# Foxhead-Studio/InsTaG

Hardware: AMD Instinct MI355X
Metric: train-step frames/sec @512x512, 100k Gaussians (higher is better)
Workload: dtype f32; 1 GPU; C3: train_face step, 100k Gaussians + 6 grid encodes + UMF/PMF motion nets (DeepSpeech feats), 512x512, SH degree 1, image + attention map in one raster pass, L1+DSSIM, Adam; targets = uniform noise (SURVEY 8d); gaussians=100000, sh_degree=1, parallelism=dp1, ranks_reported_by_backend=1, execution=hipGraph replay, timing=one window of 1714 steps after 5 warm-up steps

## Files before the change

### instag_amd/csrc/ssim.hip

```cpp
#include "common.hpp"
#include "device_math.hpp"

namespace instag {
namespace {

constexpr int TS = 16;
constexpr int RAD = 5;
constexpr int HS = TS + 2 * RAD;
constexpr float C1 = 0.01f * 0.01f;
constexpr float C2 = 0.03f * 0.03f;

__device__ constexpr float GW[11] = {0.0010283801f, 0.0075987581f, 0.0360007721f, 0.1093606895f, 0.2130055377f,
                                     0.2660117249f, 0.2130055377f, 0.1093606895f, 0.0360007721f, 0.0075987581f,
                                     0.0010283801f};

__global__ void __launch_bounds__(256)
l1_ssim_forward_kernel(const float* __restrict__ img1, const float* __restrict__ img2, int H, int W,
                       float* __restrict__ maps, float* __restrict__ part_ssim, float* __restrict__ part_l1) {
  __shared__ float s_x[HS][HS + 1], s_y[HS][HS + 1];
  __shared__ float s_h[5][HS][TS + 1];
  __shared__ float s_red[4];
  const int c = blockIdx.z;
  const int x0 = blockIdx.x * TS, y0 = blockIdx.y * TS;
  const size_t plane = (size_t)H * W;
  const float* p1 = img1 + c * plane;
  const float* p2 = img2 + c * plane;
  for (int i = threadIdx.x; i < HS * HS; i += 256) {
    const int ly = i / HS, lx = i - ly * HS;
    const int gy = y0 + ly - RAD, gx = x0 + lx - RAD;
    const bool in = gy >= 0 && gy < H && gx >= 0 && gx < W;
    s_x[ly][lx] = in ? p1[(size_t)gy * W + gx] : 0.f;
    s_y[ly][lx] = in ? p2[(size_t)gy * W + gx] : 0.f;
  }
  __syncthreads();
  for (int i = threadIdx.x; i < HS * TS; i += 256) {
    const int ly = i / TS, lx = i - ly * TS;
    float a = 0.f, b = 0.f, aa = 0.f, bb = 0.f, ab = 0.f;
#pragma unroll
    for (int k = 0; k < 11; ++k) {
      const float xv = s_x[ly][lx + k], yv = s_y[ly][lx + k], w = GW[k];
      a += w * xv; b += w * yv; aa += w * xv * xv; bb += w * yv * yv; ab += w * xv * yv;
    }
    s_h[0][ly][lx] = a; s_h[1][ly][lx] = b; s_h[2][ly][lx] = aa; s_h[3][ly][lx] = bb; s_h[4][ly][lx] = ab;
  }
  __syncthreads();
  const int tx = threadIdx.x & 15, ty = threadIdx.x >> 4;
  const int gx = x0 + tx, gy = y0 + ty;
  const bool inside = gx < W && gy < H;
  float mu1 = 0.f, mu2 = 0.f, e11 = 0.f, e22 = 0.f, e12 = 0.f;
#pragma unroll
  for (int k = 0; k < 11; ++k) {
    const float w = GW[k];
    mu1 += w * s_h[0][ty + k][tx]; mu2 += w * s_h[1][ty + k][tx];
    e11 += w * s_h[2][ty + k][tx]; e22 += w * s_h[3][ty + k][tx]; e12 += w * s_h[4][ty + k][tx];
  }
  float ssim_v = 0.f, l1_v = 0.f;
  if (inside) {
    const float mu1s = mu1 * mu1, mu2s = mu2 * mu2, mu12 = mu1 * mu2;
    const float s11 = e11 - mu1s, s22 = e22 - mu2s, s12 = e12 - mu12;
    const float A1 = 2.f * mu12 + C1, A2 = 2.f * s12 + C2, B1 = mu1s + mu2s + C1, B2 = s11 + s22 + C2;
    const float inv = 1.f / (B1 * B2);
    ssim_v = A1 * A2 * inv;
    const float dS_ds11 = -ssim_v / B2;
    const float dS_ds12 = 2.f * A1 * inv;
    const float dS_dmu1 = 2.f * mu2 * A2 * inv - 2.f * mu1 * ssim_v / B1 + dS_ds11 * (-2.f * mu1) + dS_ds12 * (-mu2);
    const size_t pix = (size_t)gy * W + gx;
    const size_t C3 = (size_t)gridDim.z * plane;
    maps[c * plane + pix] = dS_dmu1;
    maps[C3 + c * plane + pix] = dS_ds11;
    maps[2 * C3 + c * plane + pix] = dS_ds12;
    l1_v = fabsf(s_x[ty + RAD][tx + RAD] - s_y[ty + RAD][tx + RAD]);
  }
  const float bs = block_sum_256(ssim_v, s_red);
  __syncthreads();
  const float bl = block_sum_256(l1_v, s_red);
  if (threadIdx.x == 0) {
    const int bid = (blockIdx.z * gridDim.y + blockIdx.y) * gridDim.x + blockIdx.x;
    part_ssim[bid] = bs;
    part_l1[bid] = bl;
  }
}

__global__ void __launch_bounds__(256)
l1_ssim_backward_kernel(const float* __restrict__ img1, const float* __restrict__ img2,
                        const float* __restrict__ maps, const float* __restrict__ g_ssim,
                        const float* __restrict__ g_l1, int C, int H, int W, float* __restrict__ dimg1) {
  __shared__ float s_m[3][HS][HS + 1];
  __shared__ float s_h[3][HS][TS + 1];
  const int c = blockIdx.z;
  const int x0 = blockIdx.x * TS, y0 = blockIdx.y * TS;
  const size_t plane = (size_t)H * W;
  const size_t C3 = (size_t)C * plane;
  for (int i = threadIdx.x; i < HS * HS; i += 256) {
    const int ly = i / HS, lx = i - ly * HS;
    const int gy = y0 + ly - RAD, gx = x0 + lx - RAD;
    const bool in = gy >= 0 && gy < H && gx >= 0 && gx < W;
    const size_t o = c * plane + (size_t)gy * W + gx;
    s_m[0][ly][lx] = in ? maps[o] : 0.f;
    s_m[1][ly][lx] = in ? maps[C3 + o] : 0.f;
    s_m[2][ly][lx] = in ? maps[2 * C3 + o] : 0.f;
  }
  __syncthreads();
  for (int i = threadIdx.x; i < HS * TS; i += 256) {
    const int ly = i / TS, lx = i - ly * TS;
    float a = 0.f, b = 0.f, d = 0.f;
#pragma unroll
    for (int k = 0; k < 11; ++k) {
      const float w = GW[k];
      a += w * s_m[0][ly][lx + k]; b += w * s_m[1][ly][lx + k]; d += w * s_m[2][ly][lx + k];
    }
    s_h[0][ly][lx] = a; s_h[1][ly][lx] = b; s_h[2][ly][lx] = d;
  }
  __syncthreads();
  const int tx = threadIdx.x & 15, ty = threadIdx.x >> 4;
  const int gx = x0 + tx, gy = y0 + ty;
  if (gx >= W || gy >= H) return;
  float fm = 0.f, f11 = 0.f, f12 = 0.f;
#pragma unroll
  for (int k = 0; k < 11; ++k) {
    const float w = GW[k];
    fm += w * s_h[0][ty + k][tx]; f11 += w * s_h[1][ty + k][tx]; f12 += w * s_h[2][ty + k][tx];
  }
  const size_t pix = c * plane + (size_t)gy * W + gx;
  const float x = img1[pix], y = img2[pix];
  const float inv_n = 1.f / (float)C3;
  const float gs = g_ssim ? g_ssim[0] : 0.f, gl = g_l1 ? g_l1[0] : 0.f;
  const float diff = x - y;
  const float sgn = diff > 0.f ? 1.f : (diff < 0.f ? -1.f : 0.f);
  dimg1[pix] = inv_n * (gs * (fm + 2.f * x * f11 + y * f12) + gl * sgn);
}


struct FaceCfg {
  int H, W, flags;
  float w_dssim, w_alpha, w_hair, w_lips, w_extra;
};
constexpr int F_HAIR_BG = 1, F_ALPHA = 2, F_HAIR_ATTN = 4, F_LIPS = 8;
constexpr int F_MOUTH = 16;
constexpr int F_PLAIN = 32;

struct FaceIn {
  const float* image; const float* gt; const uint8_t* face; const uint8_t* hair; const uint8_t* mouth;
  const float* bg; const float* alpha; const float* attn; const int32_t* lips; const float* extra;
};

__device__ __forceinline__ bool in_lips(const FaceIn& in, int gy, int gx) {
  return gy >= in.lips[0] && gy < in.lips[1] && gx >= in.lips[2] && gx < in.lips[3];
}

__device__ __forceinline__ void face_pixel(const FaceCfg& cfg, const FaceIn& in, int c, size_t plane, size_t pix,
                                           float& x, float& y) {
  if (cfg.flags & F_PLAIN) {
    x = in.image[c * plane + pix];
    y = in.gt[c * plane + pix];
    return;
  }
  const float bgc = in.bg[c];
  if (cfg.flags & F_MOUTH) {
    const int gy = (int)(pix / (size_t)cfg.W), gx = (int)(pix - (size_t)gy * cfg.W);
    const bool mouth = in.mouth[pix] != 0, lips = in_lips(in, gy, gx);
    x = (lips != mouth) ? bgc : in.image[c * plane + pix];
    y = mouth ? in.gt[c * plane + pix] : bgc;
    return;
  }
  const bool hair = in.hair[pix] != 0, head = hair || in.face[pix] != 0, mouth = in.mouth[pix] != 0;
  const bool hair_bg = (cfg.flags & F_HAIR_BG) && hair;
  x = hair_bg ? bgc : in.image[c * plane + pix];
  y = (head && !mouth && !hair_bg) ? in.gt[c * plane + pix] : bgc;
}

__global__ void __launch_bounds__(256)
face_loss_forward_kernel(FaceCfg cfg, FaceIn in, float* __restrict__ maps, float* __restrict__ part) {
  __shared__ float s_x[HS][HS + 1], s_y[HS][HS + 1];
  __shared__ float s_h[5][HS][TS + 1];
  __shared__ float s_red[4];
  const int H = cfg.H, W = cfg.W;
  const int c = blockIdx.z;
  const int x0 = blockIdx.x * TS, y0 = blockIdx.y * TS;
  const size_t plane = (size_t)H * W;
  for (int i = threadIdx.x; i < HS * HS; i += 256) {
    const int ly = i / HS, lx = i - ly * HS;
    const int gy = y0 + ly - RAD, gx = x0 + lx - RAD;
    float xv = 0.f, yv = 0.f;
    if (gy >= 0 && gy < H && gx >= 0 && gx < W) face_pixel(cfg, in, c, plane, (size_t)gy * W + gx, xv, yv);
    s_x[ly][lx] = xv;
    s_y[ly][lx] = yv;
  }
  __syncthreads();
  for (int i = threadIdx.x; i < HS * TS; i += 256) {
    const int ly = i / TS, lx = i - ly * TS;
    float a = 0.f, b = 0.f, aa = 0.f, bb = 0.f, ab = 0.f;
#pragma unroll
    for (int k = 0; k < 11; ++k) {
      const float xv = s_x[ly][lx + k], yv = s_y[ly][lx + k], w = GW[k];
      a += w * xv; b += w * yv; aa += w * xv * xv; bb += w * yv * yv; ab += w * xv * yv;
    }
    s_h[0][ly][lx] = a; s_h[1][ly][lx] = b; s_h[2][ly][lx] = aa; s_h[3][ly][lx] = bb; s_h[4][ly][lx] = ab;
  }
  __syncthreads();
  const int tx = threadIdx.x & 15, ty = threadIdx.x >> 4;
  const int gx = x0 + tx, gy = y0 + ty;
  const bool inside = gx < W && gy < H;
  float mu1 = 0.f, mu2 = 0.f, e11 = 0.f, e22 = 0.f, e12 = 0.f;
#pragma unroll
  for (int k = 0; k < 11; ++k) {
    const float w = GW[k];
    mu1 += w * s_h[0][ty + k][tx]; mu2 += w * s_h[1][ty + k][tx];
    e11 += w * s_h[2][ty + k][tx]; e22 += w * s_h[3][ty + k][tx]; e12 += w * s_h[4][ty + k][tx];
  }
  float v[8] = {0.f, 0.f, 0.f, 0.f, 0.f, 0.f, 0.f, 0.f};
  if (inside) {
    const float mu1s = mu1 * mu1, mu2s = mu2 * mu2, mu12 = mu1 * mu2;
    const float s11 = e11 - mu1s, s22 = e22 - mu2s, s12 = e12 - mu12;
    const float A1 = 2.f * mu12 + C1, A2 = 2.f * s12 + C2, B1 = mu1s + mu2s + C1, B2 = s11 + s22 + C2;
    const float inv = 1.f / (B1 * B2);
    const float ssim_v = A1 * A2 * inv;
    const float dS_ds11 = -ssim_v / B2;
    const float dS_ds12 = 2.f * A1 * inv;
    const float dS_dmu1 = 2.f * mu2 * A2 * inv - 2.f * mu1 * ssim_v / B1 + dS_ds11 * (-2.f * mu1) + dS_ds12 * (-mu2);
    const size_t pix = (size_t)gy * W + gx;
    const size_t C3 = 3 * plane;
    maps[c * plane + pix] = dS_dmu1;
    maps[C3 + c * plane + pix] = dS_ds11;
    maps[2 * C3 + c * plane + pix] = dS_ds12;
    v[0] = ssim_v;
    v[1] = fabsf(s_x[ty + RAD][tx + RAD] - s_y[ty + RAD][tx + RAD]);
    if (c == 0) {
      const bool mouth_mode = (cfg.flags & F_MOUTH) != 0, plain = (cfg.flags & F_PLAIN) != 0;
      const bool hair = !mouth_mode && !plain && in.hair[pix] != 0;
      const bool head = plain ? false : (mouth_mode ? in_lips(in, gy, gx) : (hair || in.face[pix] != 0));
      if (cfg.flags & F_ALPHA) {
        const float a = in.alpha[pix];
        v[2] = head ? 1.f - a : 0.f;
        v[3] = head ? 0.f : a;
      }
      if ((cfg.flags & F_HAIR_ATTN) && hair) {
        v[4] = in.attn[plane + pix];
        v[5] = in.attn[pix];
        v[6] = 1.f;
      }
      if (cfg.flags & F_LIPS) {
        if (gy >= in.lips[0] && gy < in.lips[1] && gx >= in.lips[2] && gx < in.lips[3]) v[7] = in.attn[plane + pix];
      }
    }
  }
  const int tiles = gridDim.x * gridDim.y;
  const int tile = blockIdx.y * gridDim.x + blockIdx.x;
  const int nk = c == 0 ? 8 : 2;
#pragma unroll
  for (int k = 0; k < 8; ++k) {
    if (k >= nk) break;
    const float bsum = block_sum_256(v[k], s_red);
    __syncthreads();
    if (threadIdx.x == 0) {
      if (k < 2) part[(size_t)k * 3 * tiles + (size_t)c * tiles + tile] = bsum;
      else part[(size_t)6 * tiles + (size_t)(k - 2) * tiles + tile] = bsum;
    }
  }
}

__device__ __forceinline__ void face_loss_partial_sums(const float* __restrict__ part, int tiles,
                                                       const float* __restrict__ extra, int n_extra, float* s_sum,
                                                       int nwaves) {
  const int wave = threadIdx.x >> 6, lane = threadIdx.x & 63;
  for (int k = wave; k < 8; k += nwaves) {
    const float* p = k < 2 ? part + (size_t)k * 3 * tiles : part + (size_t)6 * tiles + (size_t)(k - 2) * tiles;
    const int n = k < 2 ? 3 * tiles : tiles;
    float acc = 0.f;
#pragma unroll 8
    for (int i = lane; i < n; i += 64) acc += p[i];
    acc = wave_sum(acc);
    if (lane == 0) s_sum[k] = acc;
    if (k == 7) {
      float e = 0.f;
      for (int i = lane; i < n_extra; i += 64) e += extra[i];
      e = wave_sum(e);
      if (lane == 0) s_sum[8] = e;
    }
  }
}

__device__ __forceinline__ float lips_inv_area(const FaceCfg& cfg, const int32_t* __restrict__ lips) {
  const int r0 = max(lips[0], 0), r1 = min(lips[1], cfg.H), c0 = max(lips[2], 0), c1 = min(lips[3], cfg.W);
  const float area = (float)max(r1 - r0, 0) * (float)max(c1 - c0, 0);
  return area > 0.f ? 1.f / area : 0.f;
}

__device__ __forceinline__ void face_loss_scalars(const FaceCfg& cfg, const float* s_sum, const int32_t* __restrict__ lips,
                                                  bool has_extra, float* __restrict__ out) {
  const float npix = (float)cfg.H * (float)cfg.W;
  const float l1 = s_sum[1] / (3.f * npix), ssim = s_sum[0] / (3.f * npix);
  float loss = l1 + cfg.w_dssim * (1.f - ssim);
  if (cfg.flags & F_ALPHA) loss += cfg.w_alpha * (s_sum[2] / npix + s_sum[3] / npix);
  const float inv_cnt = 1.f / fmaxf(s_sum[6], 1.f);
  if (cfg.flags & F_HAIR_ATTN) loss += cfg.w_hair * (s_sum[4] * inv_cnt + s_sum[5] * inv_cnt);
  float inv_area = 0.f;
  if (cfg.flags & F_LIPS) {
    inv_area = lips_inv_area(cfg, lips);
    loss += cfg.w_lips * s_sum[7] * inv_area;
  }
  if (has_extra) loss += cfg.w_extra * s_sum[8];
  out[0] = loss; out[1] = l1; out[2] = ssim; out[3] = inv_cnt; out[4] = inv_area;
}

__global__ void __launch_bounds__(512)
face_loss_finalize_kernel(FaceCfg cfg, const float* __restrict__ part, int tiles, const int32_t* __restrict__ lips,
                          const float* __restrict__ extra, int n_extra, float* __restrict__ out) {
  __shared__ float s_sum[9];
  face_loss_partial_sums(part, tiles, extra, n_extra, s_sum, 8);
  __syncthreads();
  if (threadIdx.x == 0) face_loss_scalars(cfg, s_sum, lips, extra != nullptr, out);
}

struct FaceFin {
  const float* part; int tiles; const float* extra; int n_extra; float* out;
};

__global__ void __launch_bounds__(256)
face_loss_backward_kernel(FaceCfg cfg, FaceIn in, const float* __restrict__ maps, const float* __restrict__ out,
                          const float* __restrict__ g_loss, const float* __restrict__ g_l1,
                          float* __restrict__ d_image, float* __restrict__ d_alpha, float* __restrict__ d_attn,
                          FaceFin fin) {
  __shared__ float s_m[3][HS][HS + 1];
  __shared__ float s_h[3][HS][TS + 1];
  __shared__ float s_sum[9];
  const int H = cfg.H, W = cfg.W;
  const int c = blockIdx.z;
  float inv_cnt = 0.f;
  if (fin.part != nullptr) {
    const bool first = blockIdx.x == 0 && blockIdx.y == 0 && c == 0;
    if (first) {
      face_loss_partial_sums(fin.part, fin.tiles, fin.extra, fin.n_extra, s_sum, 4);
      __syncthreads();
      if (threadIdx.x == 0) face_loss_scalars(cfg, s_sum, in.lips, fin.extra != nullptr, fin.out);
      inv_cnt = 1.f / fmaxf(s_sum[6], 1.f);
    } else if (c == 0 && (cfg.flags & F_HAIR_ATTN)) {
      const float* hp = fin.part + (size_t)6 * fin.tiles + (size_t)4 * fin.tiles;
      float acc = 0.f;
      for (int i = threadIdx.x; i < fin.tiles; i += 256) acc += hp[i];
      acc = block_sum_256(acc, s_sum);
      inv_cnt = 1.f / fmaxf(acc, 1.f);
    }
    __syncthreads();
  }
  const int x0 = blockIdx.x * TS, y0 = blockIdx.y * TS;
  const size_t plane = (size_t)H * W;
  const size_t C3 = 3 * plane;
  for (int i = threadIdx.x; i < HS * HS; i += 256) {
    const int ly = i / HS, lx = i - ly * HS;
    const int gy = y0 + ly - RAD, gx = x0 + lx - RAD;
    const bool inb = gy >= 0 && gy < H && gx >= 0 && gx < W;
    const size_t o = c * plane + (size_t)gy * W + gx;
    s_m[0][ly][lx] = inb ? maps[o] : 0.f;
    s_m[1][ly][lx] = inb ? maps[C3 + o] : 0.f;
    s_m[2][ly][lx] = inb ? maps[2 * C3 + o] : 0.f;
  }
  __syncthreads();
  for (int i = threadIdx.x; i < HS * TS; i += 256) {
    const int ly = i / TS, lx = i - ly * TS;
    float a = 0.f, b = 0.f, d = 0.f;
#pragma unroll
    for (int k = 0; k < 11; ++k) {
      const float w = GW[k];
      a += w * s_m[0][ly][lx + k]; b += w * s_m[1][ly][lx + k]; d += w * s_m[2][ly][lx + k];
    }
    s_h[0][ly][lx] = a; s_h[1][ly][lx] = b; s_h[2][ly][lx] = d;
  }
  __syncthreads();
  const int tx = threadIdx.x & 15, ty = threadIdx.x >> 4;
  const int gx = x0 + tx, gy = y0 + ty;
  if (gx >= W || gy >= H) return;
  float fm = 0.f, f11 = 0.f, f12 = 0.f;
#pragma unroll
  for (int k = 0; k < 11; ++k) {
    const float w = GW[k];
    fm += w * s_h[0][ty + k][tx]; f11 += w * s_h[1][ty + k][tx]; f12 += w * s_h[2][ty + k][tx];
  }
  const size_t pix = (size_t)gy * W + gx;
  float x, y;
  face_pixel(cfg, in, c, plane, pix, x, y);
  const float g = g_loss ? g_loss[0] : 0.f;
  const float gl = g + (g_l1 ? g_l1[0] : 0.f);
  const float gs = -cfg.w_dssim * g;
  const float diff = x - y;
  const float sgn = diff > 0.f ? 1.f : (diff < 0.f ? -1.f : 0.f);
  const bool mouth_mode = (cfg.flags & F_MOUTH) != 0, plain = (cfg.flags & F_PLAIN) != 0;
  const bool hair = !mouth_mode && !plain && in.hair[pix] != 0;
  const bool frozen = plain ? false
                            : (mouth_mode ? (in_lips(in, gy, gx) != (in.mouth[pix] != 0)) : ((cfg.flags & F_HAIR_BG) && hair));
  d_image[c * plane + pix] = frozen ? 0.f : (1.f / (float)C3) * (gs * (fm + 2.f * x * f11 + y * f12) + gl * sgn);
  if (c == 0) {
    const bool head = plain ? false : (mouth_mode ? in_lips(in, gy, gx) : (hair || in.face[pix] != 0));
    if (d_alpha) d_alpha[pix] = (cfg.flags & F_ALPHA) ? g * cfg.w_alpha / (float)plane * (head ? -1.f : 1.f) : 0.f;
    if (d_attn) {
      const float gh = ((cfg.flags & F_HAIR_ATTN) && hair) ? g * cfg.w_hair * (fin.part ? inv_cnt : out[3]) : 0.f;
      float gp = 0.f;
      if (cfg.flags & F_LIPS)
        if (gy >= in.lips[0] && gy < in.lips[1] && gx >= in.lips[2] && gx < in.lips[3])
          gp = g * cfg.w_lips * (fin.part ? lips_inv_area(cfg, in.lips) : out[4]);
      d_attn[pix] = gh;
      d_attn[plane + pix] = gh + gp;
      d_attn[2 * plane + pix] = 0.f;
    }
  }
}

}
}

using namespace instag;

extern "C" {

int instag_l1_ssim_num_partials(int32_t C, int32_t H, int32_t W) {
  return C * ((H + TS - 1) / TS) * ((W + TS - 1) / TS);
}

int instag_l1_ssim_forward(const float* img1, const float* img2, int32_t C, int32_t H, int32_t W, float* maps,
                           float* partial_ssim, float* partial_l1, instag_stream_t stream) {
  INSTAG_REQUIRE(img1 && img2 && maps && partial_ssim && partial_l1, "l1_ssim_forward: NULL tensor");
  INSTAG_REQUIRE(C >= 1 && C <= 65535 && H >= 1 && W >= 1, "l1_ssim_forward: bad shape");
  dim3 grid((W + TS - 1) / TS, (H + TS - 1) / TS, C);
  ProfScope p(K_LOSS_FWD, (hipStream_t)stream);
  l1_ssim_forward_kernel<<<grid, 256, 0, (hipStream_t)stream>>>(img1, img2, H, W, maps, partial_ssim, partial_l1);
  INSTAG_CHECK_LAUNCH();
  return INSTAG_OK;
}

int instag_l1_ssim_backward(const float* img1, const float* img2, const float* maps, const float* g_ssim,
                            const float* g_l1, int32_t C, int32_t H, int32_t W, float* dimg1,
                            instag_stream_t stream) {
  INSTAG_REQUIRE(img1 && img2 && maps && dimg1, "l1_ssim_backward: NULL tensor");
  INSTAG_REQUIRE(C >= 1 && C <= 65535 && H >= 1 && W >= 1, "l1_ssim_backward: bad shape");
  dim3 grid((W + TS - 1) / TS, (H + TS - 1) / TS, C);
  ProfScope p(K_LOSS_BWD, (hipStream_t)stream);
  l1_ssim_backward_kernel<<<grid, 256, 0, (hipStream_t)stream>>>(img1, img2, maps, g_ssim, g_l1, C, H, W, dimg1);
  INSTAG_CHECK_LAUNCH();
  return INSTAG_OK;
}

static int face_cfg(const instag_face_loss_cfg* c, FaceCfg* out) {
  INSTAG_REQUIRE(c, "face_loss: NULL config");
  INSTAG_REQUIRE(c->H >= 1 && c->W >= 1, "face_loss: bad image size");
  *out = FaceCfg{c->H, c->W, c->flags, c->w_dssim, c->w_alpha, c->w_attn_hair, c->w_attn_lips, c->w_extra};
  return INSTAG_OK;
}

int64_t instag_face_loss_num_partials(int32_t H, int32_t W) {
  return (int64_t)12 * ((H + TS - 1) / TS) * ((W + TS - 1) / TS);
}

static int face_loss_forward_impl(const instag_face_loss_cfg* cfg, const float* image, const float* gt,
                                  const uint8_t* face_mask, const uint8_t* hair_mask, const uint8_t* mouth_mask,
                                  const float* bg, const float* alpha, const float* attn, const int32_t* lips_rect,
                                  const float* extra, int32_t n_extra, float* maps, float* partials, float* out,
                                  bool finalize, instag_stream_t stream) {
  FaceCfg c;
  if (int rc = face_cfg(cfg, &c)) return rc;
  const bool mouth_mode = (c.flags & F_MOUTH) != 0;
  const bool plain = (c.flags & F_PLAIN) != 0;
  INSTAG_REQUIRE(image && gt && maps && partials && out, "face_loss_forward: NULL tensor");
  INSTAG_REQUIRE(plain || (mouth_mask && bg && (mouth_mode || (face_mask && hair_mask))), "face_loss_forward: NULL mask");
  INSTAG_REQUIRE(!plain || !(c.flags & ~F_PLAIN), "face_loss_forward: the plain mode takes no other term");
  INSTAG_REQUIRE(!mouth_mode || (lips_rect && !(c.flags & (F_HAIR_BG | F_HAIR_ATTN | F_LIPS))),
                 "face_loss_forward: the mouth mode needs lips_rect and none of the face-branch terms");
  INSTAG_REQUIRE(!(c.flags & F_ALPHA) || alpha, "face_loss_forward: alpha term without alpha");
  INSTAG_REQUIRE(!(c.flags & (F_HAIR_ATTN | F_LIPS)) || attn, "face_loss_forward: attention term without attn");
  INSTAG_REQUIRE(!(c.flags & F_LIPS) || lips_rect, "face_loss_forward: lips term without lips_rect");
  INSTAG_REQUIRE(extra == nullptr || n_extra >= 1, "face_loss_forward: n_extra must be >= 1");
  const FaceIn in{image, gt, face_mask, hair_mask, mouth_mask, bg, alpha, attn, lips_rect, extra};
  dim3 grid((c.W + TS - 1) / TS, (c.H + TS - 1) / TS, 3);
  {
    ProfScope p(K_LOSS_FWD, (hipStream_t)stream);
    face_loss_forward_kernel<<<grid, 256, 0, (hipStream_t)stream>>>(c, in, maps, partials);
    INSTAG_CHECK_LAUNCH();
  }
  if (!finalize) return INSTAG_OK;
  face_loss_finalize_kernel<<<1, 512, 0, (hipStream_t)stream>>>(c, partials, (int)(grid.x * grid.y), lips_rect, extra,
                                                              extra ? n_extra : 0, out);
  INSTAG_CHECK_LAUNCH();
  return INSTAG_OK;
}

int instag_face_loss_forward(const instag_face_loss_cfg* cfg, const float* image, const float* gt,
                             const uint8_t* face_mask, const uint8_t* hair_mask, const uint8_t* mouth_mask,
                             const float* bg, const float* alpha, const float* attn, const int32_t* lips_rect,
                             const float* extra, int32_t n_extra, float* maps, float* partials, float* out,
                             instag_stream_t stream) {
  return face_loss_forward_impl(cfg, image, gt, face_mask, hair_mask, mouth_mask, bg, alpha, attn, lips_rect, extra,
                                n_extra, maps, partials, out, true, stream);
}

int instag_face_loss_forward_deferred(const instag_face_loss_cfg* cfg, const float* image, const float* gt,
                                      const uint8_t* face_mask, const uint8_t* hair_mask, const uint8_t* mouth_mask,
                                      const float* bg, const float* alpha, const float* attn, const int32_t* lips_rect,
                                      const float* extra, int32_t n_extra, float* maps, float* partials,
                                      instag_stream_t stream) {
  INSTAG_REQUIRE(partials != nullptr, "face_loss_forward_deferred: NULL partials");
  float dummy = 0.f;
  return face_loss_forward_impl(cfg, image, gt, face_mask, hair_mask, mouth_mask, bg, alpha, attn, lips_rect, extra,
                                n_extra, maps, partials, &dummy, false, stream);
}

static int face_loss_backward_impl(const instag_face_loss_cfg* cfg, const float* image, const float* gt,
                                   const uint8_t* face_mask, const uint8_t* hair_mask, const uint8_t* mouth_mask,
                                   const float* bg, const int32_t* lips_rect, const float* maps, const float* out,
                                   const float* g_loss, const float* g_l1, float* d_image, float* d_alpha, float* d_attn,
                                   const FaceFin& fin, instag_stream_t stream) {
  FaceCfg c;
  if (int rc = face_cfg(cfg, &c)) return rc;
  const bool mouth_mode = (c.flags & F_MOUTH) != 0;
  const bool plain = (c.flags & F_PLAIN) != 0;
  INSTAG_REQUIRE(image && gt && maps && out && d_image, "face_loss_backward: NULL tensor");
  INSTAG_REQUIRE(plain || (mouth_mask && bg && (mouth_mode || (face_mask && hair_mask))), "face_loss_backward: NULL mask");
  INSTAG_REQUIRE(!mouth_mode || lips_rect, "face_loss_backward: the mouth mode needs lips_rect");
  INSTAG_REQUIRE(!(c.flags & F_LIPS) || lips_rect, "face_loss_backward: lips term without lips_rect");
  const FaceIn in{image, gt, face_mask, hair_mask, mouth_mask, bg, nullptr, nullptr, lips_rect, nullptr};
  dim3 grid((c.W + TS - 1) / TS, (c.H + TS - 1) / TS, 3);
  FaceFin f = fin;
  f.tiles = (int)(grid.x * grid.y);
  ProfScope p(K_LOSS_BWD, (hipStream_t)stream);
  face_loss_backward_kernel<<<grid, 256, 0, (hipStream_t)stream>>>(c, in, maps, out, g_loss, g_l1, d_image, d_alpha,
                                                                   d_attn, f);
  INSTAG_CHECK_LAUNCH();
  return INSTAG_OK;
}

int instag_face_loss_backward(const instag_face_loss_cfg* cfg, const float* image, const float* gt,
                              const uint8_t* face_mask, const uint8_t* hair_mask, const uint8_t* mouth_mask,
                              const float* bg, const int32_t* lips_rect, const float* maps, const float* out,
                              const float* g_loss, const float* g_l1, float* d_image, float* d_alpha, float* d_attn,
                              instag_stream_t stream) {
  return face_loss_backward_impl(cfg, image, gt, face_mask, hair_mask, mouth_mask, bg, lips_rect, maps, out, g_loss,
                                 g_l1, d_image, d_alpha, d_attn, FaceFin{nullptr, 0, nullptr, 0, nullptr}, stream);
}

int instag_face_loss_backward_deferred(const instag_face_loss_cfg* cfg, const float* image, const float* gt,
                                       const uint8_t* face_mask, const uint8_t* hair_mask, const uint8_t* mouth_mask,
                                       const float* bg, const int32_t* lips_rect, const float* maps,
                                       const float* partials, const float* extra, int32_t n_extra, float* out,
                                       const float* g_loss, const float* g_l1, float* d_image, float* d_alpha,
                                       float* d_attn, instag_stream_t stream) {
  INSTAG_REQUIRE(partials && out, "face_loss_backward_deferred: NULL partials / out");
  INSTAG_REQUIRE(extra == nullptr || n_extra >= 1, "face_loss_backward_deferred: n_extra must be >= 1");
  return face_loss_backward_impl(cfg, image, gt, face_mask, hair_mask, mouth_mask, bg, lips_rect, maps, out, g_loss,
                                 g_l1, d_image, d_alpha, d_attn,
                                 FaceFin{partials, 0, extra, extra ? n_extra : 0, out}, stream);
}

}
```

Before: 1065 frames/s.

## Fuse three color channels per tile in face loss forward and backward kernels

The face-loss forward and backward kernels now process all three color channels in one workgroup per tile instead of one workgroup per channel. Mask, lips and background loads happen once per tile, and halo loads are issued into registers up front. Each kernel is templated on the loss mode so per-pixel flag branches disappear. The forward reduction now uses one wave-sum pass into 12 slots, and the backward finalize scalar reduction runs in an extra dedicated workgroup rather than in tile 0. The cost is higher LDS and register use per block and a third as many blocks, which can lower occupancy.

Result: no change. 1066 frames/s (median of 4 runs) (+0.1%).

```diff
diff --git a/instag_amd/csrc/ssim.hip b/instag_amd/csrc/ssim.hip
--- a/instag_amd/csrc/ssim.hip
+++ b/instag_amd/csrc/ssim.hip
@@ -144,126 +144,187 @@
   const float* bg; const float* alpha; const float* attn; const int32_t* lips; const float* extra;
 };
 
-__device__ __forceinline__ bool in_lips(const FaceIn& in, int gy, int gx) {
-  return gy >= in.lips[0] && gy < in.lips[1] && gx >= in.lips[2] && gx < in.lips[3];
-}
-
-__device__ __forceinline__ void face_pixel(const FaceCfg& cfg, const FaceIn& in, int c, size_t plane, size_t pix,
-                                           float& x, float& y) {
-  if (cfg.flags & F_PLAIN) {
-    x = in.image[c * plane + pix];
-    y = in.gt[c * plane + pix];
-    return;
-  }
-  const float bgc = in.bg[c];
-  if (cfg.flags & F_MOUTH) {
-    const int gy = (int)(pix / (size_t)cfg.W), gx = (int)(pix - (size_t)gy * cfg.W);
-    const bool mouth = in.mouth[pix] != 0, lips = in_lips(in, gy, gx);
-    x = (lips != mouth) ? bgc : in.image[c * plane + pix];
-    y = mouth ? in.gt[c * plane + pix] : bgc;
-    return;
-  }
-  const bool hair = in.hair[pix] != 0, head = hair || in.face[pix] != 0, mouth = in.mouth[pix] != 0;
-  const bool hair_bg = (cfg.flags & F_HAIR_BG) && hair;
-  x = hair_bg ? bgc : in.image[c * plane + pix];
-  y = (head && !mouth && !hair_bg) ? in.gt[c * plane + pix] : bgc;
-}
-
+enum { M_FACE = 0, M_MOUTH = 1, M_PLAIN = 2 };
+
+constexpr int HSP = HS + 2;
+constexpr int H_ITEMS = 4 * ((HS + 7) / 8) * 32;
+__device__ __forceinline__ int h_item_row(int i) { return 8 * (i >> 7) + ((i & 31) >> 2); }
+__device__ __forceinline__ int h_item_col(int i) { return 4 * ((i >> 5) & 3) + (i & 3); }
+
+constexpr int NCELL = (HS * HS + 255) / 256;
+
+struct Lips { int r0, r1, c0, c1; };
+
+template <int MODE>
+__device__ __forceinline__ Lips load_lips(const FaceCfg& cfg, const FaceIn& in) {
+  Lips l{0, 0, 0, 0};
+  if (MODE == M_MOUTH || (MODE == M_FACE && (cfg.flags & F_LIPS))) l = Lips{in.lips[0], in.lips[1], in.lips[2], in.lips[3]};
+  return l;
+}
+
+__device__ __forceinline__ bool in_lips(const Lips& l, int gy, int gx) {
+  return gy >= l.r0 && gy < l.r1 && gx >= l.c0 && gx < l.c1;
+}
+
+struct HaloCell { int ly, lx, gy, gx; bool in; size_t pix; };
+
+__device__ __forceinline__ HaloCell halo_cell(int i, int x0, int y0, int H, int W) {
+  HaloCell h;
+  h.ly = i / HS; h.lx = i - h.ly * HS;
+  h.gy = y0 + h.ly - RAD; h.gx = x0 + h.lx - RAD;
+  h.in = i < HS * HS && h.gy >= 0 && h.gy < H && h.gx >= 0 && h.gx < W;
+  h.pix = (size_t)min(max(h.gy, 0), H - 1) * W + min(max(h.gx, 0), W - 1);
+  return h;
+}
+
+struct MaskBytes { uint8_t hair, face, mouth; };
+
+template <int MODE>
+__device__ __forceinline__ MaskBytes load_masks(const FaceIn& in, size_t pix) {
+  MaskBytes m{0, 0, 0};
+  if (MODE == M_FACE) { m.hair = in.hair[pix]; m.face = in.face[pix]; }
+  if (MODE != M_PLAIN) m.mouth = in.mouth[pix];
+  return m;
+}
+
+template <int MODE>
+__device__ __forceinline__ void face_compose(int flags, const MaskBytes& m, const Lips& l, int gy, int gx, float bgc,
+                                             float img, float gtv, float& x, float& y) {
+  if (MODE == M_PLAIN) {
+    x = img;
+    y = gtv;
+  } else if (MODE == M_MOUTH) {
+    const bool mouth = m.mouth != 0, lips = in_lips(l, gy, gx);
+    x = (lips != mouth) ? bgc : img;
+    y = mouth ? gtv : bgc;
+  } else {
+    const bool hair = m.hair != 0, head = hair || m.face != 0, mouth = m.mouth != 0;
+    const bool hair_bg = (flags & F_HAIR_BG) && hair;
+    x = hair_bg ? bgc : img;
+    y = (head && !mouth && !hair_bg) ? gtv : bgc;
+  }
+}
+
+template <int MODE>
 __global__ void __launch_bounds__(256)
 face_loss_forward_kernel(FaceCfg cfg, FaceIn in, float* __restrict__ maps, float* __restrict__ part) {
-  __shared__ float s_x[HS][HS + 1], s_y[HS][HS + 1];
-  __shared__ float s_h[5][HS][TS + 1];
-  __shared__ float s_red[4];
-  const int H = cfg.H, W = cfg.W;
-  const int c = blockIdx.z;
+  __shared__ float s_x[3][HS][HSP], s_y[3][HS][HSP];
+  __shared__ float s_h[5][HS][TS];
+  __shared__ float s_red[12][4];
+  const int H = cfg.H, W = cfg.W, flags = cfg.flags;
   const int x0 = blockIdx.x * TS, y0 = blockIdx.y * TS;
   const size_t plane = (size_t)H * W;
-  for (int i = threadIdx.x; i < HS * HS; i += 256) {
-    const int ly = i / HS, lx = i - ly * HS;
-    const int gy = y0 + ly - RAD, gx = x0 + lx - RAD;
-    float xv = 0.f, yv = 0.f;
-    if (gy >= 0 && gy < H && gx >= 0 && gx < W) face_pixel(cfg, in, c, plane, (size_t)gy * W + gx, xv, yv);
-    s_x[ly][lx] = xv;
-    s_y[ly][lx] = yv;
-  }
-  __syncthreads();
-  for (int i = threadIdx.x; i < HS * TS; i += 256) {
-    const int ly = i / TS, lx = i - ly * TS;
-    float a = 0.f, b = 0.f, aa = 0.f, bb = 0.f, ab = 0.f;
-#pragma unroll
-    for (int k = 0; k < 11; ++k) {
-      const float xv = s_x[ly][lx + k], yv = s_y[ly][lx + k], w = GW[k];
-      a += w * xv; b += w * yv; aa += w * xv * xv; bb += w * yv * yv; ab += w * xv * yv;
-    }
-    s_h[0][ly][lx] = a; s_h[1][ly][lx] = b; s_h[2][ly][lx] = aa; s_h[3][ly][lx] = bb; s_h[4][ly][lx] = ab;
-  }
-  __syncthreads();
   const int tx = threadIdx.x & 15, ty = threadIdx.x >> 4;
   const int gx = x0 + tx, gy = y0 + ty;
   const bool inside = gx < W && gy < H;
-  float mu1 = 0.f, mu2 = 0.f, e11 = 0.f, e22 = 0.f, e12 = 0.f;
-#pragma unroll
-  for (int k = 0; k < 11; ++k) {
-    const float w = GW[k];
-    mu1 += w * s_h[0][ty + k][tx]; mu2 += w * s_h[1][ty + k][tx];
-    e11 += w * s_h[2][ty + k][tx]; e22 += w * s_h[3][ty + k][tx]; e12 += w * s_h[4][ty + k][tx];
-  }
-  float v[8] = {0.f, 0.f, 0.f, 0.f, 0.f, 0.f, 0.f, 0.f};
+  const size_t cpix = (size_t)min(gy, H - 1) * W + min(gx, W - 1);
+
+  const Lips lips = load_lips<MODE>(cfg, in);
+  float bg[3] = {0.f, 0.f, 0.f};
+  if (MODE != M_PLAIN) { bg[0] = in.bg[0]; bg[1] = in.bg[1]; bg[2] = in.bg[2]; }
+  MaskBytes hm[NCELL];
+  float hx[NCELL][3], hy[NCELL][3];
+#pragma unroll
+  for (int j = 0; j < NCELL; ++j) {
+    const HaloCell h = halo_cell(threadIdx.x + 256 * j, x0, y0, H, W);
+    hm[j] = load_masks<MODE>(in, h.pix);
+#pragma unroll
+    for (int c = 0; c < 3; ++c) { hx[j][c] = in.image[c * plane + h.pix]; hy[j][c] = in.gt[c * plane + h.pix]; }
+  }
+  const float* alpha_p = (flags & F_ALPHA) ? in.alpha : in.image;
+  const float* attn_p = (flags & (F_HAIR_ATTN | F_LIPS)) ? in.attn : in.image;
+  const MaskBytes cm = load_masks<MODE>(in, cpix);
+  const float c_alpha = alpha_p[cpix], c_attn1 = attn_p[plane + cpix], c_attn0 = attn_p[cpix];
+
+#pragma unroll
+  for (int j = 0; j < NCELL; ++j) {
+    const HaloCell h = halo_cell(threadIdx.x + 256 * j, x0, y0, H, W);
+    if (j + 1 < NCELL || threadIdx.x + 256 * j < HS * HS) {
+#pragma unroll
+      for (int c = 0; c < 3; ++c) {
+        float xv, yv;
+        face_compose<MODE>(flags, hm[j], lips, h.gy, h.gx, bg[c], hx[j][c], hy[j][c], xv, yv);
+        s_x[c][h.ly][h.lx] = h.in ? xv : 0.f;
+        s_y[c][h.ly][h.lx] = h.in ? yv : 0.f;
+      }
+    }
+  }
+  __syncthreads();
+
+  float v[12] = {0.f, 0.f, 0.f, 0.f, 0.f, 0.f, 0.f, 0.f, 0.f, 0.f, 0.f, 0.f};
+#pragma unroll
+  for (int c = 0; c < 3; ++c) {
+    for (int i = threadIdx.x; i < H_ITEMS; i += 256) {
+      const int ly = h_item_row(i), lx = h_item_col(i);
+      if (ly >= HS) continue;
+      float a = 0.f, b = 0.f, aa = 0.f, bb = 0.f, ab = 0.f;
+#pragma unroll
+      for (int k = 0; k < 11; ++k) {
+        const float xv = s_x[c][ly][lx + k], yv = s_y[c][ly][lx + k], w = GW[k];
+        a += w * xv; b += w * yv; aa += w * xv * xv; bb += w * yv * yv; ab += w * xv * yv;
+      }
+      s_h[0][ly][lx] = a; s_h[1][ly][lx] = b; s_h[2][ly][lx] = aa; s_h[3][ly][lx] = bb; s_h[4][ly][lx] = ab;
+    }
+    __syncthreads();
+    float mu1 = 0.f, mu2 = 0.f, e11 = 0.f, e22 = 0.f, e12 = 0.f;
+#pragma unroll
+    for (int k = 0; k < 11; ++k) {
+      const float w = GW[k];
+      mu1 += w * s_h[0][ty + k][tx]; mu2 += w * s_h[1][ty + k][tx];
+      e11 += w * s_h[2][ty + k][tx]; e22 += w * s_h[3][ty + k][tx]; e12 += w * s_h[4][ty + k][tx];
+    }
+    if (c < 2) __syncthreads();
+    if (inside) {
+      const float mu1s = mu1 * mu1, mu2s = mu2 * mu2, mu12 = mu1 * mu2;
+      const float s11 = e11 - mu1s, s22 = e22 - mu2s, s12 = e12 - mu12;
+      const float A1 = 2.f * mu12 + C1, A2 = 2.f * s12 + C2, B1 = mu1s + mu2s + C1, B2 = s11 + s22 + C2;
+      const float inv = 1.f / (B1 * B2);
+      const float ssim_v = A1 * A2 * inv;
+      const float dS_ds11 = -ssim_v / B2;
+      const float dS_ds12 = 2.f * A1 * inv;
+      const float dS_dmu1 = 2.f * mu2 * A2 * inv - 2.f * mu1 * ssim_v / B1 + dS_ds11 * (-2.f * mu1) + dS_ds12 * (-mu2);
+      const size_t C3 = 3 * plane;
+      maps[c * plane + cpix] = dS_dmu1;
+      maps[C3 + c * plane + cpix] = dS_ds11;
+      maps[2 * C3 + c * plane + cpix] = dS_ds12;
+      v[c] = ssim_v;
+      v[3 + c] = fabsf(s_x[c][ty + RAD][tx + RAD] - s_y[c][ty + RAD][tx + RAD]);
+    }
+  }
   if (inside) {
-    const float mu1s = mu1 * mu1, mu2s = mu2 * mu2, mu12 = mu1 * mu2;
-    const float s11 = e11 - mu1s, s22 = e22 - mu2s, s12 = e12 - mu12;
-    const float A1 = 2.f * mu12 + C1, A2 = 2.f * s12 + C2, B1 = mu1s + mu2s + C1, B2 = s11 + s22 + C2;
-    const float inv = 1.f / (B1 * B2);
-    const float ssim_v = A1 * A2 * inv;
-    const float dS_ds11 = -ssim_v / B2;
-    const float dS_ds12 = 2.f * A1 * inv;
-    const float dS_dmu1 = 2.f * mu2 * A2 * inv - 2.f * mu1 * ssim_v / B1 + dS_ds11 * (-2.f * mu1) + dS_ds12 * (-mu2);
-    const size_t pix = (size_t)gy * W + gx;
-    const size_t C3 = 3 * plane;
-    maps[c * plane + pix] = dS_dmu1;
-    maps[C3 + c * plane + pix] = dS_ds11;
-    maps[2 * C3 + c * plane + pix] = dS_ds12;
-    v[0] = ssim_v;
-    v[1] = fabsf(s_x[ty + RAD][tx + RAD] - s_y[ty + RAD][tx + RAD]);
-    if (c == 0) {
-      const bool mouth_mode = (cfg.flags & F_MOUTH) != 0, plain = (cfg.flags & F_PLAIN) != 0;
-      const bool hair = !mouth_mode && !plain && in.hair[pix] != 0;
-      const bool head = plain ? false : (mouth_mode ? in_lips(in, gy, gx) : (hair || in.face[pix] != 0));
-      if (cfg.flags & F_ALPHA) {
-        const float a = in.alpha[pix];
-        v[2] = head ? 1.f - a : 0.f;
-        v[3] = head ? 0.f : a;
-      }
-      if ((cfg.flags & F_HAIR_ATTN) && hair) {
-        v[4] = in.attn[plane + pix];
-        v[5] = in.attn[pix];
-        v[6] = 1.f;
-      }
-      if (cfg.flags & F_LIPS) {
-        if (gy >= in.lips[0] && gy < in.lips[1] && gx >= in.lips[2] && gx < in.lips[3]) v[7] = in.attn[plane + pix];
-      }
-    }
-  }
-  const int tiles = gridDim.x * gridDim.y;
-  const int tile = blockIdx.y * gridDim.x + blockIdx.x;
-  const int nk = c == 0 ? 8 : 2;
-#pragma unroll
-  for (int k = 0; k < 8; ++k) {
-    if (k >= nk) break;
-    const float bsum = block_sum_256(v[k], s_red);
-    __syncthreads();
-    if (threadIdx.x == 0) {
-      if (k < 2) part[(size_t)k * 3 * tiles + (size_t)c * tiles + tile] = bsum;
-      else part[(size_t)6 * tiles + (size_t)(k - 2) * tiles + tile] = bsum;
-    }
+    const bool hair = MODE == M_FACE && cm.hair != 0;
+    const bool head = MODE == M_PLAIN ? false : (MODE == M_MOUTH ? in_lips(lips, gy, gx) : (hair || cm.face != 0));
+    if (flags & F_ALPHA) {
+      v[6] = head ? 1.f - c_alpha : 0.f;
+      v[7] = head ? 0.f : c_alpha;
+    }
+    if ((flags & F_HAIR_ATTN) && hair) {
+      v[8] = c_attn1;
+      v[9] = c_attn0;
+      v[10] = 1.f;
+    }
+    if (MODE == M_FACE && (flags & F_LIPS) && in_lips(lips, gy, gx)) v[11] = c_attn1;
+  }
+  const int wave = threadIdx.x >> 6;
+#pragma unroll
+  for (int k = 0; k < 12; ++k) v[k] = wave_sum(v[k]);
+  if ((threadIdx.x & 63) == 0) {
+#pragma unroll
+    for (int k = 0; k < 12; ++k) s_red[k][wave] = v[k];
+  }
+  __syncthreads();
+  if (threadIdx.x < 12) {
+    const int tiles = gridDim.x * gridDim.y;
+    const int tile = blockIdx.y * gridDim.x + blockIdx.x;
+    const float* r = s_red[threadIdx.x];
+    part[(size_t)threadIdx.x * tiles + tile] = ((r[0] + r[1]) + r[2]) + r[3];
   }
 }
 
 __device__ __forceinline__ void face_loss_partial_sums(const float* __restrict__ part, int tiles,
-                                                       const float* __restrict__ extra, int n_extra, float* s_sum,
-                                                       int nwaves) {
+                                                       const float* __restrict__ extra, int n_extra, float* s_sum) {
   const int wave = threadIdx.x >> 6, lane = threadIdx.x & 63;
-  for (int k = wave; k < 8; k += nwaves) {
+  if (const int k = wave; k < 8) {
     const float* p = k < 2 ? part + (size_t)k * 3 * tiles : part + (size_t)6 * tiles + (size_t)(k - 2) * tiles;
     const int n = k < 2 ? 3 * tiles : tiles;
     float acc = 0.f;
@@ -307,7 +368,7 @@
 face_loss_finalize_kernel(FaceCfg cfg, const float* __restrict__ part, int tiles, const int32_t* __restrict__ lips,
                           const float* __restrict__ extra, int n_extra, float* __restrict__ out) {
   __shared__ float s_sum[9];
-  face_loss_partial_sums(part, tiles, extra, n_extra, s_sum, 8);
+  face_loss_partial_sums(part, tiles, extra, n_extra, s_sum);
   __syncthreads();
   if (threadIdx.x == 0) face_loss_scalars(cfg, s_sum, lips, extra != nullptr, out);
 }
@@ -316,88 +377,156 @@
   const float* part; int tiles; const float* extra; int n_extra; float* out;
 };
 
+template <int CH>
+__device__ __forceinline__ float lane_strided_sum(const float* __restrict__ p, int n, int lane) {
+  float acc = 0.f;
+  for (int base = lane; base < n; base += 64 * CH) {
+    float r[CH];
+#pragma unroll
+    for (int u = 0; u < CH; ++u) r[u] = p[min(base + 64 * u, n - 1)];
+#pragma unroll
+    for (int u = 0; u < CH; ++u)
+      if (base + 64 * u < n) acc += r[u];
+  }
+  return acc;
+}
+
+__device__ __forceinline__ void face_loss_scalar_workgroup(const FaceCfg& cfg, const int32_t* __restrict__ lips,
+                                                           const FaceFin& fin, float* s_sum) {
+  const int wave = threadIdx.x >> 6, lane = threadIdx.x & 63;
+  const int tiles = fin.tiles;
+  for (int k = wave; k < 8; k += 4) {
+    const float* p = k < 2 ? fin.part + (size_t)k * 3 * tiles : fin.part + (size_t)6 * tiles + (size_t)(k - 2) * tiles;
+    const float acc = wave_sum(k < 2 ? lane_strided_sum<48>(p, 3 * tiles, lane) : lane_strided_sum<16>(p, tiles, lane));
+    if (lane == 0) s_sum[k] = acc;
+    if (k == 7) {
+      const float e = wave_sum(lane_strided_sum<16>(fin.extra, fin.n_extra, lane));
+      if (lane == 0) s_sum[8] = e;
+    }
+  }
+  __syncthreads();
+  if (threadIdx.x == 0) face_loss_scalars(cfg, s_sum, lips, fin.extra != nullptr, fin.out);
+}
+
+__device__ __forceinline__ float loss_grad_pixel(float inv_n, float gs, float gl, float fm, float f11, float f12, float x,
+                                                 float y, float sgn) {
+#pragma clang fp contract(off)
+  return inv_n * (gs * (fm + 2.f * x * f11 + y * f12) + gl * sgn);
+}
+
+template <int MODE>
 __global__ void __launch_bounds__(256)
 face_loss_backward_kernel(FaceCfg cfg, FaceIn in, const float* __restrict__ maps, const float* __restrict__ out,
                           const float* __restrict__ g_loss, const float* __restrict__ g_l1,
                           float* __restrict__ d_image, float* __restrict__ d_alpha, float* __restrict__ d_attn,
-                          FaceFin fin) {
-  __shared__ float s_m[3][HS][HS + 1];
-  __shared__ float s_h[3][HS][TS + 1];
+                          FaceFin fin, int tiles_x) {
+  __shared__ float s_m[9][HS][HSP];
+  __shared__ float s_h[3][HS][TS];
   __shared__ float s_sum[9];
-  const int H = cfg.H, W = cfg.W;
-  const int c = blockIdx.z;
-  float inv_cnt = 0.f;
-  if (fin.part != nullptr) {
-    const bool first = blockIdx.x == 0 && blockIdx.y == 0 && c == 0;
-    if (first) {
-      face_loss_partial_sums(fin.part, fin.tiles, fin.extra, fin.n_extra, s_sum, 4);
-      __syncthreads();
-      if (threadIdx.x == 0) face_loss_scalars(cfg, s_sum, in.lips, fin.extra != nullptr, fin.out);
-      inv_cnt = 1.f / fmaxf(s_sum[6], 1.f);
-    } else if (c == 0 && (cfg.flags & F_HAIR_ATTN)) {
-      const float* hp = fin.part + (size_t)6 * fin.tiles + (size_t)4 * fin.tiles;
-      float acc = 0.f;
-      for (int i = threadIdx.x; i < fin.tiles; i += 256) acc += hp[i];
-      acc = block_sum_256(acc, s_sum);
-      inv_cnt = 1.f / fmaxf(acc, 1.f);
-    }
-    __syncthreads();
-  }
-  const int x0 = blockIdx.x * TS, y0 = blockIdx.y * TS;
+  if ((int)blockIdx.x == fin.tiles) {
+    face_loss_scalar_workgroup(cfg, in.lips, fin, s_sum);
+    return;
+  }
+  const int H = cfg.H, W = cfg.W, flags = cfg.flags;
+  const int by = blockIdx.x / tiles_x, bx = blockIdx.x - by * tiles_x;
+  const int x0 = bx * TS, y0 = by * TS;
   const size_t plane = (size_t)H * W;
   const size_t C3 = 3 * plane;
-  for (int i = threadIdx.x; i < HS * HS; i += 256) {
-    const int ly = i / HS, lx = i - ly * HS;
-    const int gy = y0 + ly - RAD, gx = x0 + lx - RAD;
-    const bool inb = gy >= 0 && gy < H && gx >= 0 && gx < W;
-    const size_t o = c * plane + (size_t)gy * W + gx;
-    s_m[0][ly][lx] = inb ? maps[o] : 0.f;
-    s_m[1][ly][lx] = inb ? maps[C3 + o] : 0.f;
-    s_m[2][ly][lx] = inb ? maps[2 * C3 + o] : 0.f;
-  }
-  __syncthreads();
-  for (int i = threadIdx.x; i < HS * TS; i += 256) {
-    const int ly = i / TS, lx = i - ly * TS;
-    float a = 0.f, b = 0.f, d = 0.f;
-#pragma unroll
-    for (int k = 0; k < 11; ++k) {
-      const float w = GW[k];
-      a += w * s_m[0][ly][lx + k]; b += w * s_m[1][ly][lx + k]; d += w * s_m[2][ly][lx + k];
-    }
-    s_h[0][ly][lx] = a; s_h[1][ly][lx] = b; s_h[2][ly][lx] = d;
-  }
-  __syncthreads();
   const int tx = threadIdx.x & 15, ty = threadIdx.x >> 4;
   const int gx = x0 + tx, gy = y0 + ty;
-  if (gx >= W || gy >= H) return;
-  float fm = 0.f, f11 = 0.f, f12 = 0.f;
-#pragma unroll
-  for (int k = 0; k < 11; ++k) {
-    const float w = GW[k];
-    fm += w * s_h[0][ty + k][tx]; f11 += w * s_h[1][ty + k][tx]; f12 += w * s_h[2][ty + k][tx];
-  }
-  const size_t pix = (size_t)gy * W + gx;
-  float x, y;
-  face_pixel(cfg, in, c, plane, pix, x, y);
+  const bool inside = gx < W && gy < H;
+  const size_t pix = (size_t)min(gy, H - 1) * W + min(gx, W - 1);
+  const bool deferred = fin.part != nullptr;
+
   const float g = g_loss ? g_loss[0] : 0.f;
   const float gl = g + (g_l1 ? g_l1[0] : 0.f);
   const float gs = -cfg.w_dssim * g;
-  const float diff = x - y;
-  const float sgn = diff > 0.f ? 1.f : (diff < 0.f ? -1.f : 0.f);
-  const bool mouth_mode = (cfg.flags & F_MOUTH) != 0, plain = (cfg.flags & F_PLAIN) != 0;
-  const bool hair = !mouth_mode && !plain && in.hair[pix] != 0;
-  const bool frozen = plain ? false
-                            : (mouth_mode ? (in_lips(in, gy, gx) != (in.mouth[pix] != 0)) : ((cfg.flags & F_HAIR_BG) && hair));
-  d_image[c * plane + pix] = frozen ? 0.f : (1.f / (float)C3) * (gs * (fm + 2.f * x * f11 + y * f12) + gl * sgn);
-  if (c == 0) {
-    const bool head = plain ? false : (mouth_mode ? in_lips(in, gy, gx) : (hair || in.face[pix] != 0));
-    if (d_alpha) d_alpha[pix] = (cfg.flags & F_ALPHA) ? g * cfg.w_alpha / (float)plane * (head ? -1.f : 1.f) : 0.f;
+  const Lips lips = load_lips<MODE>(cfg, in);
+  float bg[3] = {0.f, 0.f, 0.f};
+  if (MODE != M_PLAIN) { bg[0] = in.bg[0]; bg[1] = in.bg[1]; bg[2] = in.bg[2]; }
+  const bool hair_term = MODE == M_FACE && (flags & F_HAIR_ATTN) && d_attn != nullptr;
+  const bool lips_term = MODE == M_FACE && (flags & F_LIPS) && d_attn != nullptr;
+  float inv_cnt = (hair_term && !deferred) ? out[3] : 0.f;
+  const float inv_area = lips_term ? (deferred ? lips_inv_area(cfg, in.lips) : out[4]) : 0.f;
+  const bool count = hair_term && deferred;
+  const float* hp = count ? fin.part + (size_t)6 * fin.tiles + (size_t)4 * fin.tiles : maps;
+  float hc[4];
+#pragma unroll
+  for (int u = 0; u < 4; ++u) hc[u] = hp[min((int)threadIdx.x + 256 * u, fin.tiles - 1)];
+  float hm[NCELL][9];
+#pragma unroll
+  for (int j = 0; j < NCELL; ++j) {
+    const HaloCell h = halo_cell(threadIdx.x + 256 * j, x0, y0, H, W);
+#pragma unroll
+    for (int q = 0; q < 9; ++q) hm[j][q] = maps[(q % 3) * C3 + (q / 3) * plane + h.pix];
+  }
+  const MaskBytes cm = load_masks<MODE>(in, pix);
+  float ci[3], cg[3];
+#pragma unroll
+  for (int c = 0; c < 3; ++c) { ci[c] = in.image[c * plane + pix]; cg[c] = in.gt[c * plane + pix]; }
+
+  if (count) {
+    float cnt = 0.f;
+#pragma unroll
+    for (int u = 0; u < 4; ++u)
+      if ((int)threadIdx.x + 256 * u < fin.tiles) cnt += hc[u];
+    for (int i = threadIdx.x + 1024; i < fin.tiles; i += 256) cnt += hp[i];
+    cnt = wave_sum(cnt);
+    if ((threadIdx.x & 63) == 0) s_sum[threadIdx.x >> 6] = cnt;
+  }
+#pragma unroll
+  for (int j = 0; j < NCELL; ++j) {
+    const HaloCell h = halo_cell(threadIdx.x + 256 * j, x0, y0, H, W);
+    if (j + 1 < NCELL || threadIdx.x + 256 * j < HS * HS) {
+#pragma unroll
+      for (int q = 0; q < 9; ++q) s_m[q][h.ly][h.lx] = h.in ? hm[j][q] : 0.f;
+    }
+  }
+  __syncthreads();
+  if (count) inv_cnt = 1.f / fmaxf(((s_sum[0] + s_sum[1]) + s_sum[2]) + s_sum[3], 1.f);
+
+  const bool hair = MODE == M_FACE && cm.hair != 0;
+  const bool frozen = MODE == M_PLAIN ? false
+                                      : (MODE == M_MOUTH ? (in_lips(lips, gy, gx) != (cm.mouth != 0))
+                                                         : ((flags & F_HAIR_BG) && hair));
+#pragma unroll
+  for (int c = 0; c < 3; ++c) {
+    for (int i = threadIdx.x; i < H_ITEMS; i += 256) {
+      const int ly = h_item_row(i), lx = h_item_col(i);
+      if (ly >= HS) continue;
+      float a = 0.f, b = 0.f, d = 0.f;
+#pragma unroll
+      for (int k = 0; k < 11; ++k) {
+        const float w = GW[k];
+        a = __fmaf_rn(w, s_m[3 * c][ly][lx + k], a); b = __fmaf_rn(w, s_m[3 * c + 1][ly][lx + k], b);
+        d = __fmaf_rn(w, s_m[3 * c + 2][ly][lx + k], d);
+      }
+      s_h[0][ly][lx] = a; s_h[1][ly][lx] = b; s_h[2][ly][lx] = d;
+    }
+    __syncthreads();
+    float fm = 0.f, f11 = 0.f, f12 = 0.f;
+#pragma unroll
+    for (int k = 0; k < 11; ++k) {
+      const float w = GW[k];
+      fm = __fmaf_rn(w, s_h[0][ty + k][tx], fm); f11 = __fmaf_rn(w, s_h[1][ty + k][tx], f11);
+      f12 = __fmaf_rn(w, s_h[2][ty + k][tx], f12);
+    }
+    if (c < 2) __syncthreads();
+    if (inside) {
+      float x, y;
+      face_compose<MODE>(flags, cm, lips, gy, gx, bg[c], ci[c], cg[c], x, y);
+      const float diff = x - y;
+      const float sgn = diff > 0.f ? 1.f : (diff < 0.f ? -1.f : 0.f);
+      d_image[c * plane + pix] = frozen ? 0.f : loss_grad_pixel(1.f / (float)C3, gs, gl, fm, f11, f12, x, y, sgn);
+    }
+  }
+  if (inside) {
+    const bool head = MODE == M_PLAIN ? false : (MODE == M_MOUTH ? in_lips(lips, gy, gx) : (hair || cm.face != 0));
+    if (d_alpha) d_alpha[pix] = (flags & F_ALPHA) ? g * cfg.w_alpha / (float)plane * (head ? -1.f : 1.f) : 0.f;
     if (d_attn) {
-      const float gh = ((cfg.flags & F_HAIR_ATTN) && hair) ? g * cfg.w_hair * (fin.part ? inv_cnt : out[3]) : 0.f;
+      const float gh = ((flags & F_HAIR_ATTN) && hair) ? g * cfg.w_hair * inv_cnt : 0.f;
       float gp = 0.f;
-      if (cfg.flags & F_LIPS)
-        if (gy >= in.lips[0] && gy < in.lips[1] && gx >= in.lips[2] && gx < in.lips[3])
-          gp = g * cfg.w_lips * (fin.part ? lips_inv_area(cfg, in.lips) : out[4]);
+      if (lips_term && in_lips(lips, gy, gx)) gp = g * cfg.w_lips * inv_area;
       d_attn[pix] = gh;
       d_attn[plane + pix] = gh + gp;
       d_attn[2 * plane + pix] = 0.f;
@@ -469,10 +598,12 @@
   INSTAG_REQUIRE(!(c.flags & F_LIPS) || lips_rect, "face_loss_forward: lips term without lips_rect");
   INSTAG_REQUIRE(extra == nullptr || n_extra >= 1, "face_loss_forward: n_extra must be >= 1");
   const FaceIn in{image, gt, face_mask, hair_mask, mouth_mask, bg, alpha, attn, lips_rect, extra};
-  dim3 grid((c.W + TS - 1) / TS, (c.H + TS - 1) / TS, 3);
+  dim3 grid((c.W + TS - 1) / TS, (c.H + TS - 1) / TS);
   {
     ProfScope p(K_LOSS_FWD, (hipStream_t)stream);
-    face_loss_forward_kernel<<<grid, 256, 0, (hipStream_t)stream>>>(c, in, maps, partials);
+    if (plain) face_loss_forward_kernel<M_PLAIN><<<grid, 256, 0, (hipStream_t)stream>>>(c, in, maps, partials);
+    else if (mouth_mode) face_loss_forward_kernel<M_MOUTH><<<grid, 256, 0, (hipStream_t)stream>>>(c, in, maps, partials);
+    else face_loss_forward_kernel<M_FACE><<<grid, 256, 0, (hipStream_t)stream>>>(c, in, maps, partials);
     INSTAG_CHECK_LAUNCH();
   }
   if (!finalize) return INSTAG_OK;
@@ -516,12 +647,14 @@
   INSTAG_REQUIRE(!mouth_mode || lips_rect, "face_loss_backward: the mouth mode needs lips_rect");
   INSTAG_REQUIRE(!(c.flags & F_LIPS) || lips_rect, "face_loss_backward: lips term without lips_rect");
   const FaceIn in{image, gt, face_mask, hair_mask, mouth_mask, bg, nullptr, nullptr, lips_rect, nullptr};
-  dim3 grid((c.W + TS - 1) / TS, (c.H + TS - 1) / TS, 3);
+  const int tiles_x = (c.W + TS - 1) / TS, tiles_y = (c.H + TS - 1) / TS;
   FaceFin f = fin;
-  f.tiles = (int)(grid.x * grid.y);
+  f.tiles = tiles_x * tiles_y;
+  const dim3 grid(f.tiles + (f.part != nullptr ? 1 : 0));
   ProfScope p(K_LOSS_BWD, (hipStream_t)stream);
-  face_loss_backward_kernel<<<grid, 256, 0, (hipStream_t)stream>>>(c, in, maps, out, g_loss, g_l1, d_image, d_alpha,
-                                                                   d_attn, f);
+  auto kernel = plain ? face_loss_backward_kernel<M_PLAIN>
+                      : (mouth_mode ? face_loss_backward_kernel<M_MOUTH> : face_loss_backward_kernel<M_FACE>);
+  kernel<<<grid, 256, 0, (hipStream_t)stream>>>(c, in, maps, out, g_loss, g_l1, d_image, d_alpha, d_attn, f, tiles_x);
   INSTAG_CHECK_LAUNCH();
   return INSTAG_OK;
 }
```
